# ThibHlln/smartpy

Measured on AMD Instinct MI355X. Metric: MC sample-timesteps/sec/GPU; 1e5 LHS x hourly 10-yr forcing, higher is better.
Workload: dtype f64

## Files before the change

include/smart_amd.h:

```cpp
#ifndef SMART_AMD_H
#define SMART_AMD_H

#include <stdint.h>

#ifdef __cplusplus
extern "C" {
#endif

#define SMART_AMD_ABI_VERSION 7

#define SMART_REPORT_SUMMARY 1
#define SMART_REPORT_RAW 2

#define SMART_MATH_LITERAL 0
#define SMART_MATH_FAST 1

#define SMART_OK 0
#define SMART_E_NULL (-1)
#define SMART_E_SIZE (-2)
#define SMART_E_REPORT_TYPE (-3)
#define SMART_E_WARMUP (-4)
#define SMART_E_GAP (-5)
#define SMART_E_NO_DEVICE (-6)
#define SMART_E_MODE (-7)
// ... 7 lines not shown
#define SMART_PLAN_FORCING_VARYING 0x20
#define SMART_PLAN_FORCING_RUNS 0x80
#define SMART_PLAN_ROWS_ORDERED 0x40
#define SMART_PLAN_VALID 0x100
#define SMART_PLAN_ILLCOND_BLOCKS_SHIFT 12
#define SMART_PLAN_ILLCOND_BLOCKS_MAX 0x7ffff

#define SMART_LITERAL_FORM_AUTO 0
#define SMART_LITERAL_FORM_ROWS 1
#define SMART_LITERAL_FORM_LANES 2

#define SMART_STATUS_SLICE_TIMEOUT 0x1
#define SMART_STATUS_STALE_PLAN 0x2
#define SMART_STATUS_NONFINITE_FORCING 0x4

typedef struct SmartEnsemble {
    int64_t n_catchments;
    int64_t n_samples;
    int64_t n_steps;
    int64_t n_warm;
    int64_t report_gap;
    int32_t report_type;
    int32_t math_mode;
    double delta_sec;

    const double *area_m2;
    const double *forcing;
    const double *params;
    int64_t params_catchment_stride;
    const double *extra;
// ... 2 lines not shown
    const double *gw_obs;

    double *discharge;
    int64_t discharge_ld;
    double *gw;
    double *objfn;
    double *final_vars;
    void *workspace;
    int64_t workspace_bytes;

    void *stream;

    int32_t time_slices;
    int32_t plan;
    int32_t literal_form;
    int32_t reserved0;
} SmartEnsemble;

int64_t smart_n_reports(int64_t n_steps, int64_t report_gap, int32_t report_type);

int smart_run_ensemble_hip(const SmartEnsemble *e);

int smart_check_ensemble(const SmartEnsemble *e);

int64_t smart_workspace_bytes(const SmartEnsemble *e);

int smart_plan_ensemble(const SmartEnsemble *e, int32_t *plan);

int smart_launch_status(const SmartEnsemble *e, int32_t *status);

int smart_describe_launch(const SmartEnsemble *e, char *text, int64_t len);

int smart_allsteps_hip(double area_m2, double delta_sec, int64_t length_simu, const double *nd_rain,
                       const double *nd_peva, const double *nd_parameters, const double *nd_initial,
                       int32_t report_type, int64_t report_gap, double *discharge,
                       double *groundwater_component, double *final_vars);

int smart_hook_counters(int64_t *counters, int64_t n);
// ... 160 lines not shown
```

smartpy_amd/_lib.py:

```python
import contextlib
import ctypes
import os

_HERE = os.path.dirname(os.path.abspath(__file__))
LIB_PATH = os.environ.get('SMART_AMD_LIB') or os.path.join(_HERE, 'csrc', 'libsmart_amd.so')

REPORT_SUMMARY, REPORT_RAW = 1, 2
MATH_LITERAL, MATH_FAST = 0, 1
ABI_VERSION = 7
PLAN_VALID = 0x100
PLAN_CLASS_BITS = {0: 0x01, 1: 0x02, 2: 0x04, 3: 0x08}
PLAN_FORCING_PIECEWISE, PLAN_FORCING_VARYING, PLAN_FORCING_RUNS = 0x10, 0x20, 0x80
PLAN_ROWS_ORDERED = 0x40
PLAN_ILLCOND_BLOCKS_SHIFT, PLAN_ILLCOND_BLOCKS_MAX = 12, 0x7ffff
LITERAL_FORM_AUTO, LITERAL_FORM_ROWS, LITERAL_FORM_LANES = 0, 1, 2
STATUS_SLICE_TIMEOUT, STATUS_STALE_PLAN, STATUS_NONFINITE_FORCING = 0x1, 0x2, 0x4
QUANTILES_AUTO, QUANTILES_SORT, QUANTILES_SELECT = 0, 1, 2
QUANTILES_MAX_PROBS = 16
TRANSFORMS = {'none': 0, 'sqrt': 1, 'log': 2, 'inverse': 3}
OBJFN_WINDOW_COLS = 7
FDC_METHODS = {'auto': 0, 'sort': 1, 'select': 2}
SIGNATURE_NAMES = ['MEAN', 'BFI', 'FLASHINESS', 'AC1', 'RLD', 'RECESSION', 'PEAK', 'PEAK_ROW', 'HIGH_COUNT',
                   'HIGH_DURATION', 'LOW_COUNT', 'LOW_DURATION']
SIGNATURE_COLS = len(SIGNATURE_NAMES)
BOOT_MEAN, BOOT_STD = 0, 1
SOBOL_MAX_PARAMS = 16
PARETO_MAX_OBJECTIVES = 16
PARETO_DIRECTIONS = {'max': 0, 'min': 1, 'target': 2}
ENSEMBLE_SCORE_NAMES = ['CRPS', 'SPREAD', 'PIT_LOW', 'PIT_HIGH', 'MEAN']
ENSEMBLE_SCORE_COLS = len(ENSEMBLE_SCORE_NAMES)
ENSEMBLE_METHODS = {'auto': 0, 'lds': 1, 'global': 2}
# ... 3 lines not shown
PAWN_METHODS = {'auto': 0, 'lds': 1, 'global': 2}

_dp = ctypes.c_void_p


class SmartEnsemble(ctypes.Structure):
    _fields_ = [
        ('n_catchments', ctypes.c_int64), ('n_samples', ctypes.c_int64), ('n_steps', ctypes.c_int64),
        ('n_warm', ctypes.c_int64), ('report_gap', ctypes.c_int64),
        ('report_type', ctypes.c_int32), ('math_mode', ctypes.c_int32), ('delta_sec', ctypes.c_double),
        ('area_m2', _dp), ('forcing', _dp), ('params', _dp), ('params_catchment_stride', ctypes.c_int64),
        ('extra', _dp), ('initial', _dp), ('obs', _dp), ('gw_obs', _dp),
        ('discharge', _dp), ('discharge_ld', ctypes.c_int64), ('gw', _dp), ('objfn', _dp),
        ('final_vars', _dp), ('workspace', _dp), ('workspace_bytes', ctypes.c_int64), ('stream', _dp),
        ('time_slices', ctypes.c_int32), ('plan', ctypes.c_int32),
        ('literal_form', ctypes.c_int32), ('reserved0', ctypes.c_int32),
    ]


SYMBOLS = {
    'smart_n_reports': (ctypes.c_int64, [ctypes.c_int64, ctypes.c_int64, ctypes.c_int32]),
    'smart_run_ensemble_hip': (ctypes.c_int, [ctypes.POINTER(SmartEnsemble)]),
    'smart_check_ensemble': (ctypes.c_int, [ctypes.POINTER(SmartEnsemble)]),
    'smart_workspace_bytes': (ctypes.c_int64, [ctypes.POINTER(SmartEnsemble)]),
    'smart_plan_ensemble': (ctypes.c_int, [ctypes.POINTER(SmartEnsemble), ctypes.POINTER(ctypes.c_int32)]),
    'smart_launch_status': (ctypes.c_int, [ctypes.POINTER(SmartEnsemble), ctypes.POINTER(ctypes.c_int32)]),
    'smart_describe_launch': (ctypes.c_int, [ctypes.POINTER(SmartEnsemble), ctypes.c_char_p, ctypes.c_int64]),
    'smart_allsteps_hip': (ctypes.c_int, [ctypes.c_double, ctypes.c_double, ctypes.c_int64, _dp, _dp, _dp, _dp,
                                          ctypes.c_int32, ctypes.c_int64, _dp, _dp, _dp]),
    'smart_hook_counters': (ctypes.c_int, [ctypes.POINTER(ctypes.c_int64), ctypes.c_int64]),
    'smart_onestep_hip': (ctypes.c_int, [ctypes.c_int64, _dp, _dp]),
    'smart_river_step_hip': (ctypes.c_int, [ctypes.c_int64, _dp, _dp]),
    'smart_objfn_hip': (ctypes.c_int, [ctypes.c_int64, ctypes.c_int64, _dp, ctypes.c_int64, _dp, _dp,
                                       ctypes.c_double, _dp, _dp]),
    'smart_weighted_quantiles_hip': (ctypes.c_int, [ctypes.c_int64, ctypes.c_int64, _dp, ctypes.c_int64, _dp,
                                                    ctypes.POINTER(ctypes.c_double), ctypes.c_int32, _dp,
                                                    ctypes.c_int32, _dp]),
    'smart_quantiles_sort_capacity': (ctypes.c_int64, []),
# ... 122 lines not shown
```

smartpy_amd/csrc/smart_capi.hip:

```cpp
#include "smart_capi_internal.h"
#include "smart_fast_entry.h"

#include <cmath>
#include <cstdarg>
#include <cstdio>
#include <cstdlib>
#include <cstring>
#include <mutex>
#include <vector>

namespace smart {

static_assert(kStatusSliceTimeout == SMART_STATUS_SLICE_TIMEOUT && kStatusStalePlan == SMART_STATUS_STALE_PLAN,
              "status bits of smart_device.h and include/smart_amd.h");

static thread_local char g_err[512] = "";

int fail(int code, const char *fmt, ...)
{
    va_list ap;
    va_start(ap, fmt);
    vsnprintf(g_err, sizeof(g_err), fmt, ap);
    va_end(ap);
    return code;
// ... 55 lines not shown
                    r[4 * j] = f[t].x;
                    r[4 * j + 1] = f[t].y;
                    r[4 * j + 2] = obs && dev && rr >= 0 && rr < a.R ? obs[rr] : 0.0;
                    r[4 * j + 3] = obs && dev && rr >= 0 && rr < a.R ? dev[rr] : 0.0;
                }
                code = a.gap == 1 ? every_code(p, step_kind(f[2 * p]), step_kind(f[2 * p + 1]))
                                  : gap_code(p, a.gap, step_kind(f[2 * p]), step_kind(f[2 * p + 1]));
            }
            for (int j = 0; j < 8; ++j)
                rec[p * 8 + j] = r[j];
            codes[p] = code;
        }
    }
    if (bad)
        __hip_atomic_fetch_or(a.fflags + blockIdx.y, bad, __ATOMIC_RELAXED, __HIP_MEMORY_SCOPE_AGENT);
    if (wild && a.hdr)
        __hip_atomic_fetch_or(a.hdr + kHdrStatus, kStatusNonFiniteForcing, __ATOMIC_RELAXED, __HIP_MEMORY_SCOPE_AGENT);
}

__global__ void smart_workspace_reset(int *hdr, long n_hdr, int *flags, long n_flags)
{
    const long i = (long)blockIdx.x * blockDim.x + threadIdx.x;
    if (i < n_hdr)
        hdr[i] = 0;
    if (i < n_flags)
        flags[i] = 0;
}

__global__ __launch_bounds__(kWave) void smart_classify_rows(KArgs a)
{
    const int cls = wave_class(a, (long)blockIdx.x, (long)blockIdx.y);
    if (threadIdx.x == 0) {
        __hip_atomic_fetch_or(a.hdr + kHdrPlan, 1 << cls, __ATOMIC_RELAXED, __HIP_MEMORY_SCOPE_AGENT);
        if (cls == 3)
            __hip_atomic_fetch_add(a.hdr + kHdrPlanIllCond, 1, __ATOMIC_RELAXED, __HIP_MEMORY_SCOPE_AGENT);
    }
}

__global__ void smart_classify_forcing(KArgs a, int *hdr)
{
    const long c = (long)blockIdx.x * blockDim.x + threadIdx.x;
    if (c < a.n_catch) {
        const int kind = forcing_kind(a, a.fflags[c]);
        __hip_atomic_fetch_or(hdr + kHdrPlan,
                              kind == kForcingIntervals ? SMART_PLAN_FORCING_PIECEWISE
                                                        : (kind == kForcingRuns ? SMART_PLAN_FORCING_RUNS
                                                                                : SMART_PLAN_FORCING_VARYING),
                              __ATOMIC_RELAXED, __HIP_MEMORY_SCOPE_AGENT);
    }
}

constexpr int kMaxDevices = 64, kMaxTodo = 8, kMaxAux = kMaxTodo - 1;

struct DeviceCtx {
    std::once_flag once;
    int n_simd = 0;
    std::mutex mu;
    hipStream_t aux[kMaxAux] = {};
    hipEvent_t fork = nullptr, join[kMaxAux] = {};
    size_t lds_size[kNumFastKernels][17] = {};
    bool lds_known[kNumFastKernels][17] = {};
};

static DeviceCtx g_dev[kMaxDevices];

static DeviceCtx *device_ctx()
{
    int dev = 0;
    if (hipGetDevice(&dev) != hipSuccess || dev < 0 || dev >= kMaxDevices)
        return nullptr;
    DeviceCtx *d = &g_dev[dev];
    std::call_once(d->once, [d, dev] {
        int cus = 0;
        if (hipDeviceGetAttribute(&cus, hipDeviceAttributeMultiprocessorCount, dev) == hipSuccess && cus > 0)
            d->n_simd = cus * 4;
    });
// ... 181 lines not shown
    if (e->params_catchment_stride != 0 && e->params_catchment_stride < e->n_samples * 10)
        return fail(SMART_E_SIZE, "params_catchment_stride must be 0 or >= n_samples * 10");
    if (e->discharge && e->discharge_ld < e->n_samples)
        return fail(SMART_E_SIZE, "discharge_ld must be >= n_samples");
    if (e->objfn && (!e->obs || !e->workspace))
        return fail(SMART_E_NULL, "objfn needs obs and workspace");
    if (e->objfn && e->workspace_bytes < (int64_t)layout(e, false).state_off)
        return fail(SMART_E_SIZE, "workspace_bytes %lld is less than the %lld the header and the observation statistics need",
                    (long long)e->workspace_bytes, (long long)layout(e, false).state_off);
    if (e->time_slices < 0)
        return fail(SMART_E_SIZE, "time_slices must be >= 0");
    if (e->plan != 0 && !(e->plan & SMART_PLAN_VALID))
        return fail(SMART_E_SIZE, "plan must be 0 or a value returned by smart_plan_ensemble");
    if (e->literal_form < SMART_LITERAL_FORM_AUTO || e->literal_form > SMART_LITERAL_FORM_LANES)
        return fail(SMART_E_MODE, "literal_form must be SMART_LITERAL_FORM_AUTO, _ROWS or _LANES");
    clear_error();
    return SMART_OK;
}

int device_ready()
{
    int n = 0;
    hipError_t err = hipGetDeviceCount(&n);
    if (err != hipSuccess)
        return hip_fail(err, "hipGetDeviceCount");
    if (n < 1)
        return fail(SMART_E_NO_DEVICE, "no HIP device is visible; this engine has no CPU fallback");
    return SMART_OK;
}

// ... 94 lines not shown
    a.initial = e->initial;
    a.obs = e->obs;
    a.gw_obs = e->gw_obs;
    a.ws = e->objfn ? w.stats : nullptr;
    a.discharge = e->discharge;
    a.ld = e->discharge_ld;
    a.gw = e->gw;
    a.objfn = e->objfn;
    a.final_vars = e->final_vars;
    a.np_mean = e->math_mode == SMART_MATH_LITERAL && e->report_type == SMART_REPORT_SUMMARY && a.gap >= 8 && a.gap <= 128;
    a.pair_stride = e->final_vars ? (int)kPairStrideSplit : (int)kPairStride;
    a.n_catch = e->n_catchments;
    a.n_blocks = (a.N + kWave - 1) / kWave;
    a.seg_blocks = a.n_blocks * a.n_catch;
    a.hdr = w.hdr;
    a.fflags = nullptr;
    const int merged = merged_report(e);
    if ((merged == kReportMean || merged == kReportLast) && a.gap <= 0x7fffffff) {
        for (long q = 1; q * q <= a.gap && a.n_div < kMaxDiv; ++q)
            if (a.gap % q == 0 && a.gap / q >= 2)
                a.div[a.n_div++] = (int)(a.gap / q);
        for (long q = (long)std::sqrt((double)a.gap) + 1; q >= 2 && a.n_div < kMaxDiv; --q)
            if (q * q < a.gap && a.gap % q == 0 && q < a.div[a.n_div - 1])
                a.div[a.n_div++] = (int)q;
    }
    return a;
}

static void reset_workspace(const Workspace &w, long n_catch, int *flags, long n_flags, hipStream_t s)
{
    const long n_hdr = kHdrInts + n_catch, n = n_hdr > n_flags ? n_hdr : n_flags;
    hipLaunchKernelGGL(smart_workspace_reset, dim3((unsigned)((n + 255) / 256)), dim3(256), 0, s, w.hdr, n_hdr, flags,
                       n_flags);
}

static void set_codes(KArgs *a, const Workspace &w, const Overrides &ov)
{
    a->codes = nullptr, a->estream = nullptr, a->ecodes = nullptr;
    if (!w.codes || !pair_blocks_wanted(ov))
        return;
    if (w.lay.ecodes_off != w.lay.codes_off) {
        a->estream = (const double *)w.codes;
        a->ecodes = (const unsigned *)(w.codes + (w.lay.ecodes_off - w.lay.codes_off));
    } else {
        a->codes = (const uint2 *)w.codes;
    }
}

static void scan_forcing(const SmartEnsemble *e, KArgs a, const Workspace &w, const Overrides &ov, hipStream_t s)
{
    a.fflags = w.fflags;
    set_codes(&a, w, ov);
    hipLaunchKernelGGL(smart_forcing_scan, dim3(64, (unsigned)e->n_catchments), dim3(256), 0, s, a,
                       reinterpret_cast<const double2 *>(e->forcing));
}

static hipError_t launch_kernel(FastKernel k, KArgs a, dim3 grid, size_t lds, hipStream_t s)
{
    const double2 *forcing = reinterpret_cast<const double2 *>(a.forcing);
    const double *obs = a.obs, *ws = a.ws;
    void *args[] = {&a, &forcing, &obs, &ws};
    return hipLaunchKernel(kFastKernels[k].handle, grid, dim3(kWave), args, lds, s);
}

struct Decision {
    FastKernel todo[kMaxTodo];
    int n_todo = 0;
    bool overflow = false;
    void push(FastKernel k)
// ... 86 lines not shown
        return fail(SMART_E_SIZE, "the plan names no class of rows");
    return SMART_OK;
}

static int run(const SmartEnsemble *e, const Overrides &ov, bool literal_rows = false)
{
    int rc = check(e);
    if (rc)
        return rc;
    if ((rc = device_ready()))
        return rc;
    hipStream_t s = (hipStream_t)e->stream;
    const Workspace w = carve(e, ov);
    KArgs a = kernel_args(e, w);

    if (e->objfn)
        hipLaunchKernelGGL(smart_obs_prepare, dim3((unsigned)e->n_catchments), dim3(256), 0, s, e->obs, a.R, w.stats);

    const dim3 grid((unsigned)a.n_blocks, (unsigned)e->n_catchments);
    if (e->math_mode == SMART_MATH_LITERAL) {
        if (w.hdr)
            reset_workspace(w, e->n_catchments, nullptr, 0, s);
        a.hdr = nullptr;
        launch_literal(a, grid, a.np_mean ? (size_t)a.gap * kWave * sizeof(double) : 0, s, literal_rows);
        HIP_TRY(hipGetLastError());
        return SMART_OK;
    }

    DeviceCtx *d = device_ctx();
    if (!d)
        return fail(SMART_E_NO_DEVICE, "cannot query the current HIP device");
    Decision x;
    if ((rc = decide(e, d, w, ov, &x)))
        return rc;
    const int n_seg = x.n_seg, n_todo = x.n_todo;
    a.exits = x.exits;
    a.class_mask = x.class_mask;
    a.pc_mask = x.pc_mask;

    KArgs a_sliced = a;
    if (n_seg > 1) {
        a_sliced.n_seg = n_seg;
        a_sliced.taper = ov.taper && slice_taper_applies(a.W / a.gap + a.R, n_seg);
        a_sliced.seg_state = (double *)w.state;
        a_sliced.seg_flag = (int *)(w.state + (w.lay.flags_off - w.lay.state_off));
        a_sliced.max_polls = ov.max_polls;
        a_sliced.debug_drop = ov.drop_slice;
#ifdef SMART_SLICE_TIMELINE
        a_sliced.timeline = (unsigned long long *)w.timeline;
#endif
    }
    if (w.hdr) {
        reset_workspace(w, e->n_catchments, a_sliced.seg_flag, n_seg > 1 ? a.seg_blocks : 0, s);
        scan_forcing(e, a, w, ov, s);
        if (x.report >= 0 && (x.class_mask & SMART_PLAN_CLASS_REGULAR)) {
            a.fflags = a_sliced.fflags = w.fflags;
            set_codes(&a, w, ov);
            a_sliced.codes = a.codes, a_sliced.estream = a.estream, a_sliced.ecodes = a.ecodes;
        }
    }

    std::lock_guard<std::mutex> lock(d->mu);
    auto launch = [&](FastKernel k, hipStream_t st) -> hipError_t {
        if (kFastKernels[k].sliced && n_seg > 1) {
            const size_t lds = x.per_simd <= 3 ? lds_for_residency(d, k, 4 * x.per_simd) : 0;
            return launch_kernel(k, a_sliced, dim3((unsigned)(a.seg_blocks * n_seg), 1), lds, st);
        }
        return launch_kernel(k, a, dim3(grid.x * kFastKernels[k].waves, grid.y), 0, st);
    };
// ... 70 lines not shown
static int make_plan(const SmartEnsemble *e, const Overrides &ov, int32_t *plan)
{
    if (!plan)
        return fail(SMART_E_NULL, "smart_plan_ensemble: plan is NULL");
    *plan = 0;
    int rc = check(e);
    if (rc)
        return rc;
    if ((rc = device_ready()))
        return rc;
    const Workspace w = carve(e, ov);
    if (!w.hdr)
        return fail(SMART_E_NULL, "smart_plan_ensemble needs a workspace of smart_workspace_bytes() bytes");
    hipStream_t s = (hipStream_t)e->stream;
    KArgs a = kernel_args(e, w);
    reset_workspace(w, e->n_catchments, nullptr, 0, s);
    hipLaunchKernelGGL(smart_classify_rows, dim3((unsigned)a.n_blocks, (unsigned)e->n_catchments), dim3(kWave), 0, s, a);
    if (merged_report(e) == kReportMean || merged_report(e) == kReportLast) {
        scan_forcing(e, a, w, ov, s);
        a.fflags = w.fflags;
        hipLaunchKernelGGL(smart_classify_forcing, dim3((unsigned)((e->n_catchments + 255) / 256)), dim3(256), 0, s,
                           a, w.hdr);
    }
    HIP_TRY(hipGetLastError());
    int bits[2] = {0, 0};
    static_assert(kHdrPlanIllCond == kHdrPlan + 1, "read back together");
    HIP_TRY(hipMemcpyAsync(bits, w.hdr + kHdrPlan, sizeof(bits), hipMemcpyDeviceToHost, s));
    HIP_TRY(hipStreamSynchronize(s));
    const long n_ill = bits[1] < 0 ? 0 : (bits[1] > SMART_PLAN_ILLCOND_BLOCKS_MAX ? SMART_PLAN_ILLCOND_BLOCKS_MAX : bits[1]);
    *plan = SMART_PLAN_VALID | (bits[0] & (0x3f | SMART_PLAN_FORCING_RUNS)) |
            (int32_t)(n_ill << SMART_PLAN_ILLCOND_BLOCKS_SHIFT);
    return SMART_OK;
}

static int launch_status(const SmartEnsemble *e, int32_t *status)
{
    if (!e || !status)
        return fail(SMART_E_NULL, "smart_launch_status: NULL argument");
    *status = 0;
    if (!e->workspace || e->workspace_bytes < (int64_t)layout(e, false).header)
        return SMART_OK;
    int rc = device_ready();
    if (rc)
        return rc;
    int word = 0;
    HIP_TRY(hipMemcpyAsync(&word, (const int *)e->workspace + kHdrStatus, sizeof(int), hipMemcpyDeviceToHost,
// ... 217 lines not shown
}

using namespace smart;

extern "C" {

int64_t smart_n_reports(int64_t n_steps, int64_t report_gap, int32_t report_type)
{
    if (report_gap < 1 || n_steps < 0)
        return 0;
    return report_type == SMART_REPORT_RAW ? (n_steps + report_gap - 1) / report_gap : n_steps / report_gap;
}

int smart_check_ensemble(const SmartEnsemble *e) { return check(e); }

int64_t smart_workspace_bytes(const SmartEnsemble *e) { return workspace_bytes(e, read_overrides()); }

int smart_run_ensemble_hip(const SmartEnsemble *e) { return run(e, read_overrides()); }

int smart_plan_ensemble(const SmartEnsemble *e, int32_t *plan) { return make_plan(e, read_overrides(), plan); }

int smart_launch_status(const SmartEnsemble *e, int32_t *status) { return launch_status(e, status); }

int smart_describe_launch(const SmartEnsemble *e, char *text, int64_t len)
{
    return describe(e, read_overrides(), text, len);
}

int smart_allsteps_hip(double area_m2, double delta_sec, int64_t length_simu, const double *nd_rain,
                       const double *nd_peva, const double *nd_parameters, const double *nd_initial,
// ... 106 lines not shown
```

smartpy_amd/csrc/smart_device.h:

```cpp
#pragma once

#include "smart_slice_cuts.h"
#include "smart_matrix_common.h"

#include <hip/hip_runtime.h>

#include <type_traits>

namespace smart {

constexpr int kMaxDiv = 12;
constexpr int kForcingInsane = 1 << 30;

struct KArgs {
    long N, T, W, gap, R, first_len;
    int report_type;
    int np_mean;
    double dt;
    const double *area;
    const double *forcing;
    const double *params;
    long pstride_c;
    const double *extra;
    const double *initial;
// ... 13 lines not shown
    const double *estream = nullptr;
    const unsigned *ecodes = nullptr;
    int pair_stride = 0;
    const uint2 *codes = nullptr;
    int n_div = 0;
    int div[kMaxDiv] = {};
    int n_seg = 1;
    int taper = 0;
    long n_catch = 1;
    long n_blocks = 0;
    long seg_blocks = 0;
    double *seg_state = nullptr;
    int *seg_flag = nullptr;
    long max_polls = 0;
    int debug_drop = 0;
#ifdef SMART_SLICE_TIMELINE
    unsigned long long *timeline = nullptr;
#endif
};
#ifdef SMART_SLICE_TIMELINE
constexpr int kTimelineFields = 5, kTimelineSlices = 64;
__device__ __forceinline__ void timeline_note(const KArgs &a, long block, long c, int seg, int field,
                                              unsigned long long value)
{
    if (a.timeline && a.n_seg > 1 && seg < kTimelineSlices && seg < a.n_seg && threadIdx.x == 0)
        a.timeline[((long)seg * a.seg_blocks + c * a.n_blocks + block) * kTimelineFields + field] = value;
}
#endif

enum SegField : int {
// ... 2 lines not shown
    kSegPend = 15,
    kSegOutflows = 16,
    kSegA = 17,
    kSegB,
    kSegC1,
    kSegC2,
    kSegC3,
    kSegShift,
    kSegFields
};
enum HdrInt : int {
    kHdrStatus = 0,
    kHdrTicket = 1,
    kHdrPlan = 8,
    kHdrPlanIllCond = 9,
    kHdrInts = 64
};
constexpr int kStatusSliceTimeout = 1, kStatusStalePlan = 2, kStatusNonFiniteForcing = 4;

__device__ __forceinline__ void raise_status(const KArgs &a, int bit)
{
    if (a.hdr && threadIdx.x == 0)
        __hip_atomic_fetch_or(a.hdr + kHdrStatus, bit, __ATOMIC_RELAXED, __HIP_MEMORY_SCOPE_AGENT);
}

#define SMART_NOPS_0 ""
#define SMART_NOPS_1 "s_nop 0\n\t"
#define SMART_NOPS_2 SMART_NOPS_1 SMART_NOPS_1
#define SMART_NOPS_4 SMART_NOPS_2 SMART_NOPS_2
#define SMART_NOPS_8 SMART_NOPS_4 SMART_NOPS_4
// ... 524 lines not shown
                add_moments(val, e, w);
        }
    }
};

template <class Model>
__device__ __forceinline__ void write_results(const KArgs &a, const LaneCtx &x, const Model &m, const Reporter &rep,
                                              double gw, const double *flows = nullptr)
{
    if (x.live)
        a.gw[x.c * a.N + x.n] = gw;
    if (rep.want_obj && x.live) {
        double o[8];
        finish_objectives(rep.ws, rep.A, rep.B, rep.C1, rep.C2, rep.C3, gw, a.gw_obs ? a.gw_obs[x.c] : quiet_nan(),
                          o);
        double *op = a.objfn + (x.c * a.N + x.n) * 8;
#pragma unroll
        for (int i = 0; i < 8; ++i)
            op[i] = o[i];
    }
    if (a.final_vars) {
        double v[19];
        m.get_vars(v, flows);
        if (x.live) {
            double *fp = a.final_vars + (x.c * a.N + x.n) * 19;
#pragma unroll
            for (int i = 0; i < 19; ++i)
                fp[i] = v[i];
        }
    }
}

template <class Model, bool NP_MEAN>
__device__ __forceinline__ void run_ensemble(const KArgs &a, const double2 *__restrict__ forcing,
// ... 444 lines not shown
    [[maybe_unused]] const double *__restrict__ dev_c = ws_all ? ws_all + x.c * (kWsHead + a.R) + kWsHead : nullptr;
    [[maybe_unused]] const uint2 *codes_c = a.codes ? a.codes + x.c * code_chunks(a.T) : nullptr;
    [[maybe_unused]] const double2 *f_asm = reinterpret_cast<const double2 *>(a.forcing) + x.c * a.T;
    double num = 0.0, den = 0.0, q_out_total = 0.0;
    [[maybe_unused]] double num_raw = 0.0, den_raw = 0.0;
    double *hand = a.seg_state + (slot * kSegFields) * kWave + x.lane;
    if (seg > 0) {
        if (!wait_for_slice(a, slot, seg)) {
            const double nan = quiet_nan();
            if (a.discharge && x.live)
                for (long r = ra; r < rb; ++r)
                    a.discharge[(x.c * a.R + r) * a.ld + x.n] = nan;
            if (last) {
                if (x.live) {
                    a.gw[x.c * a.N + x.n] = nan;
                    if (a.objfn)
                        for (int i = 0; i < 8; ++i)
                            a.objfn[(x.c * a.N + x.n) * 8 + i] = nan;
                    if (a.final_vars)
                        for (int i = 0; i < 19; ++i)
                            a.final_vars[(x.c * a.N + x.n) * 19 + i] = nan;
                }
            } else {
                publish_slice(a, slot, seg, false);
            }
            return;
        }
#ifdef SMART_SLICE_TIMELINE
        timeline_note(a, block, catchment, seg, 3, __builtin_amdgcn_s_memrealtime());
#endif
        m.load_state(hand, kWave);
        if constexpr (REPORT == kReportLast) {
            num_raw = hand[kSegOutflows * kWave];
// ... 354 lines not shown
```

smartpy_amd/distributed.py:

```python
import os
import threading
import time
from datetime import timedelta

import torch
import torch.distributed as dist



def shard_bounds(n_rows, world_size, rank):
    per = -(-n_rows // world_size)
    lo = min(rank * per, n_rows)
    return lo, min(lo + per, n_rows)


def shard_counts(n_rows, world_size):
    return [shard_bounds(n_rows, world_size, r)[1] - shard_bounds(n_rows, world_size, r)[0]
            for r in range(world_size)]


def env_world():
    return (int(os.environ.get('RANK', '0')), int(os.environ.get('WORLD_SIZE', '1')),
            int(os.environ.get('LOCAL_RANK', '0')))

# ... 237 lines not shown

class ShardedEnsemble(object):

    def __init__(self, params, forcing, area_m2, delta_sec, n_warm, report_gap, axis='samples', n_catchments=None,
                 obs=None, gw_obs=None, extra=None, device=None, local_block=False, **kw):
        import numpy as np
        from . import engine
        rank, world = rank_world()
        self.axis = axis
        self.device = torch.device(device) if device is not None else engine.default_device()
        if axis == 'samples':
            self.n_total = params.shape[0] * (world if local_block else 1)
            lo, hi = (0, params.shape[0]) if local_block else shard_bounds(self.n_total, world, rank)
            self.n_local = hi - lo
            local_params = params[lo:hi] if hi > lo else params[:1]
            self._prep = engine.prepare_ensemble(local_params, forcing, area_m2, delta_sec, n_warm, report_gap,
                                                 obs=obs, gw_obs=gw_obs, extra=extra, device=self.device, **kw)
            n_run = local_params.shape[0]
            tail = (9,)
        elif axis == 'catchments':
            C = int(n_catchments if n_catchments is not None else forcing.shape[0])
            self.n_total = C
            lo, hi = shard_bounds(C, world, rank)
            self.n_local = hi - lo
            cs = list(range(lo, hi)) if hi > lo else [0]

            def per_catchment(x, shared_ndim):
                if x is None or isinstance(x, dict) or np.ndim(x) <= shared_ndim:
                    return x
                return x[cs]
            f_local = np.stack([np.asarray(forcing(c), dtype=np.float64) for c in cs]) if callable(forcing) \
                else forcing[cs]
            self._prep = engine.prepare_ensemble(
                per_catchment(params, 2), f_local, per_catchment(area_m2, 0), delta_sec, n_warm, report_gap,
                obs=per_catchment(obs, 1), gw_obs=per_catchment(gw_obs, 0), extra=per_catchment(extra, 1),
                device=self.device, **kw)
            n_run = len(cs)
            tail = (params.shape[-2], 9)
        else:
            raise Exception("axis must be 'samples' or 'catchments'")
        per = -(-self.n_total // world)
        self._packed = torch.full((max(per, n_run),) + tail, float('nan'), dtype=torch.float64, device=self.device)
        self._n_run = n_run
        self._gathered = torch.empty((world * per,) + tail, dtype=torch.float64, device=self.device) \
            if is_distributed() and not _host_staged() else None

    def step(self):
        self._prep.enqueue()
        return self._pack_and_gather(self._prep.result())

    def _pack_and_gather(self, out):
        k = self.n_local
        if k:
            if self.axis == 'samples':
                if out.objfn is not None:
                    self._packed[:k, :8].copy_(out.objfn[:k])
                self._packed[:k, 8].copy_(out.gw[:k])
            else:
                objfn = out.objfn if out.objfn is None or out.objfn.dim() == 3 else out.objfn.unsqueeze(0)
                gw = out.gw if out.gw.dim() == 2 else out.gw.unsqueeze(0)
                if objfn is not None:
                    self._packed[:k, :, :8].copy_(objfn[:k])
                self._packed[:k, :, 8].copy_(gw[:k])
        per = -(-self.n_total // rank_world()[1])
        return gather_rows(self._packed[:per], self.n_total, out=self._gathered)

    def verify(self):
        from .engine import SmartEngineError
# ... 42 lines not shown
```

smartpy_amd/engine.py:

```python
import collections
import ctypes
import math
import threading
import warnings
import weakref

import numpy as np
import torch

from . import _lib
from ._lib import SmartEngineError, REPORT_SUMMARY, REPORT_RAW, MATH_LITERAL, MATH_FAST

OBJ_FN_NAMES = ['NSE', 'KGE', 'KGEc', 'KGEa', 'KGEb', 'PBias', 'RMSE', 'GW']
VARIABLES = ['Q_aeva', 'Q_ove', 'Q_dra', 'Q_int', 'Q_sgw', 'Q_dgw', 'Q_out',
             'V_ove', 'V_dra', 'V_int', 'V_sgw', 'V_dgw',
             'V_ly1', 'V_ly2', 'V_ly3', 'V_ly4', 'V_ly5', 'V_ly6', 'V_river']

_REPORT = {'summary': REPORT_SUMMARY, 'raw': REPORT_RAW}
_MATH = {'literal': MATH_LITERAL, 'fast': MATH_FAST}
_LITERAL_FORMS = {'auto': _lib.LITERAL_FORM_AUTO, 'rows': _lib.LITERAL_FORM_ROWS, 'lanes': _lib.LITERAL_FORM_LANES}


def report_code(report):
    try:
# ... 161 lines not shown
def _compose_plan(planned, keep=0, row_class=None):
    if row_class is not None:
        forcing = _lib.PLAN_FORCING_PIECEWISE | _lib.PLAN_FORCING_VARYING | _lib.PLAN_FORCING_RUNS
        return _lib.PLAN_VALID | (planned & forcing) | _lib.PLAN_CLASS_BITS[row_class]
    return planned | (keep & _lib.PLAN_ROWS_ORDERED)


class PreparedEnsemble(object):

    repeated = False

    def __init__(self, e, device, n_samples, squeeze, outputs, workspace, grouping, caller_out, keep, memo):
        self._e = e
        self.device, self.n_samples, self._squeeze = device, n_samples, squeeze
        self._dis, self._gw, self._objfn, self._fin = outputs
        self._ws = workspace
        self._grouping = grouping
        self._caller_out = caller_out
        self._keep = keep
        self._memo = memo

    @property
    def has_status(self):
        return self._ws is not None and self._e.math_mode == MATH_FAST

    def enqueue(self):
        with torch.cuda.device(self.device):
            self._e.stream = torch.cuda.current_stream(self.device).cuda_stream
            _lib.check(_lib.lib().smart_run_ensemble_hip(ctypes.byref(self._e)))

    def launch(self):
        self.enqueue()
        return self._result()

    def result(self):
        return self._result()

    def status(self):
        word = ctypes.c_int32(0)
        with torch.cuda.device(self.device):
            self._e.stream = torch.cuda.current_stream(self.device).cuda_stream
            _lib.check(_lib.lib().smart_launch_status(ctypes.byref(self._e), ctypes.byref(word)))
        return int(word.value)

# ... 12 lines not shown
            word, ' + '.join(n for b, n in ((_lib.STATUS_SLICE_TIMEOUT, 'a time slice timed out'),
                                            (_lib.STATUS_STALE_PLAN, 'stale plan'),
                                            (_lib.STATUS_NONFINITE_FORCING, 'a NaN or an infinity in the forcing'))
                             if word & b),
            'in literal arithmetic' if word & _lib.STATUS_NONFINITE_FORCING else (
                'without time slices' if word & _lib.STATUS_SLICE_TIMEOUT else 'with a fresh plan')))
        if word & _lib.STATUS_NONFINITE_FORCING:
            self._e.math_mode = MATH_LITERAL
        if word & _lib.STATUS_SLICE_TIMEOUT:
            self._e.time_slices = 1
        if word & _lib.STATUS_STALE_PLAN:
            self._memo.forget()
            self._memo.refresh()
            self._plan()
            self._memo.store((self._grouping, int(self._e.plan)))
        self.enqueue()
        word = self.status()
        if word != 0:
            raise SmartEngineError(-6, "smartpy_amd: the repeated launch reports status %#x as well" % word)
        return self._result()

    def _plan(self, ordered=0):
        keep, word = self._e.plan | ordered, ctypes.c_int32(0)
        self._e.plan = 0
        with torch.cuda.device(self.device):
            self._e.stream = torch.cuda.current_stream(self.device).cuda_stream
            _lib.check(_lib.lib().smart_plan_ensemble(ctypes.byref(self._e), ctypes.byref(word)))
        self._e.plan = _compose_plan(int(word.value), keep)

    def aim_at(self, row_class):
        self._e.plan = _compose_plan(self._e.plan, row_class=row_class)

    def _result(self):
        dis, gw, objfn, fin = self._dis, self._gw, self._objfn, self._fin
        if self._grouping is not None:
            inverse = self._grouping[1]
            gw = gw[:, inverse]
            objfn = None if objfn is None else objfn[:, inverse]
            fin = None if fin is None else fin[:, inverse]
# ... 21 lines not shown
        raise Exception("params [C, N, 10] must have one block per catchment")
    if params.shape[-1] != 10:
        raise Exception("params must have 10 columns (T, C, H, D, S, Z, SK, FK, GK, RK)")
    pstride = 0 if params.dim() == 2 else params.shape[1] * 10
    rtype = report_code(report)
    try:
        mmode = _MATH[math_mode]
    except KeyError:
        raise Exception("math mode '{}' unknown.".format(math_mode))
    if mmode == MATH_FAST and not (isinstance(forcing_in, torch.Tensor) and forcing_in.is_cuda):
        if not bool(np.isfinite(np.asarray(forcing_in, dtype=np.float64)).all()):
            mmode = MATH_LITERAL
    return device, params, forcing, squeeze, pstride, rtype, mmode


def _allocate_outputs(C, R, N, device, want_discharge, want_objfn, want_final, discharge_out):
    dis = discharge_out
    if dis is not None:
        assert dis.is_contiguous() and dis.dtype == torch.float64 and dis.shape[:2] == (C, R) and dis.shape[2] >= N
    elif want_discharge:
        dis = torch.empty((C, R, N), dtype=torch.float64, device=device)
    return (dis, torch.empty((C, N), dtype=torch.float64, device=device),
            torch.empty((C, N, 8), dtype=torch.float64, device=device) if want_objfn else None,
            torch.empty((C, N, 19), dtype=torch.float64, device=device) if want_final else None)


def _fill_struct(inputs, outputs, pstride, n_warm, report_gap, rtype, mmode, delta_sec, time_slices, literal_form):
    def ptr(t):
        return None if t is None else t.data_ptr()

    forcing, params, dis = inputs[1], inputs[2], outputs[0]
    e = _lib.SmartEnsemble()
    e.n_catchments, e.n_samples, e.n_steps, e.n_warm = forcing.shape[0], params.shape[-2], forcing.shape[1], int(n_warm)
    e.report_gap, e.report_type, e.math_mode, e.delta_sec = int(report_gap), rtype, mmode, float(delta_sec)
    e.area_m2, e.forcing, e.params, e.extra, e.initial, e.obs, e.gw_obs = [ptr(t) for t in inputs]
    e.discharge, e.gw, e.objfn, e.final_vars = [ptr(t) for t in outputs]
    e.discharge_ld = params.shape[-2] if dis is None else dis.shape[2]
    e.params_catchment_stride, e.time_slices = pstride, int(time_slices)
    try:
        e.literal_form = _LITERAL_FORMS[literal_form]
    except KeyError:
        raise Exception("literal_form '{}' unknown ('auto', 'rows' or 'lanes').".format(literal_form))
    return e


def _size_workspace(e, device):
    with torch.cuda.device(device):
        n_ws = int(_lib.lib().smart_workspace_bytes(ctypes.byref(e)))
    ws = torch.empty((n_ws + 7) // 8, dtype=torch.float64, device=device) if n_ws > 0 else None
    e.workspace, e.workspace_bytes = (None if ws is None else ws.data_ptr()), n_ws
    _lib.check(_lib.lib().smart_check_ensemble(ctypes.byref(e)))
    return ws


def prepare_ensemble(params, forcing, area_m2, delta_sec, n_warm, report_gap, report='summary', extra=None,
                     initial=None, obs=None, gw_obs=None, math_mode='fast', want_discharge=True, want_objfn=None,
                     want_final=False, device=None, discharge_out=None, group_variants=True, time_slices=0,
                     literal_form='auto'):
    _lib.lib()
    inputs_in = (params, forcing)
    device, params, forcing, squeeze, pstride, rtype, mmode = _normalise_inputs(params, forcing, report, math_mode, device)
    C, T, N = forcing.shape[0], forcing.shape[1], params.shape[-2]
    R = n_reports(T, report_gap, rtype)
    area = _per_catchment(area_m2, device, C)
    extra = _per_catchment(extra_vector(extra) if isinstance(extra, dict) else extra, device, C, (7,))
    initial = _per_catchment(initial, device, C, (N, 12))
    if want_objfn is None:
        want_objfn = obs is not None
    if want_objfn and obs is None:
        raise Exception("objective functions need observations")
    obs = _per_catchment(obs, device, C, (R,))
    gw_obs = _per_catchment(gw_obs, device, C)

    sort_rows = not want_discharge and discharge_out is None
    memo = _Memo(inputs_in, (float(delta_sec), int(report_gap), rtype, C, N, T, bool(group_variants), sort_rows),
                 device, initial, mmode == MATH_FAST)
    known = memo.lookup()
    grouping, caller_out = None, None
    if group_variants and mmode == MATH_FAST and pstride == 0 and N > 64:
        grouping = known[0] if known else _variant_grouping(params, float(delta_sec), sort_rows, initial, area)
    if grouping is not None:
        params = params[grouping[0]].contiguous()
        initial = None if initial is None else initial[:, grouping[0]].contiguous()
    if grouping is not None and discharge_out is not None:
        caller_out, discharge_out, want_discharge = discharge_out, None, True
    outputs = _allocate_outputs(C, R, params.shape[-2], device, want_discharge, want_objfn, want_final, discharge_out)
    inputs = (area, forcing, params, extra, initial, obs, gw_obs)
    e = _fill_struct(inputs, outputs, pstride, n_warm, report_gap, rtype, mmode, delta_sec, time_slices, literal_form)
    p = PreparedEnsemble(e, device, N, squeeze, outputs, _size_workspace(e, device), grouping, caller_out, inputs, memo)
    if p.has_status:
        if known:
            e.plan = known[1]
        elif not torch.cuda.is_current_stream_capturing():
            p._plan(_lib.PLAN_ROWS_ORDERED if (sort_rows and grouping is not None) else 0)
            memo.store((grouping, int(e.plan)))
    return p


def run_ensemble(params, forcing, area_m2, delta_sec, n_warm, report_gap, report='summary', extra=None,
                 initial=None, obs=None, gw_obs=None, math_mode='fast', want_discharge=True, want_objfn=None,
                 want_final=False, device=None, discharge_out=None, group_variants=True, time_slices=0, verify=True,
                 literal_form='auto'):
    p = prepare_ensemble(params, forcing, area_m2, delta_sec, n_warm, report_gap, report=report, extra=extra,
                         initial=initial, obs=obs, gw_obs=gw_obs, math_mode=math_mode,
                         want_discharge=want_discharge, want_objfn=want_objfn, want_final=want_final, device=device,
                         discharge_out=discharge_out, group_variants=group_variants, time_slices=time_slices,
                         literal_form=literal_form)
    p.enqueue()
    out = p.verify() if verify and p.has_status and not torch.cuda.is_current_stream_capturing() else p.result()
    out._prepared = p
# ... 93 lines not shown
```

Measured before the change: 957.0 billion.

## Cache forcing scan and obs preparation across launches; write packed results directly

Adds a prepare-inputs entry point that runs the observation preparation and forcing scan once and records them per workspace. Later launches skip those kernels when forcing and obs have not changed, and the nonfinite-forcing status is carried in a kept header slot. Separately, a packed-results flag lets the kernel write objectives plus groundwater into a 9-wide caller buffer, so the distributed gather no longer needs its copy step. The cost is extra host bookkeeping and the risk of stale cached state if inputs change without a version bump.

```diff
diff --git a/include/smart_amd.h b/include/smart_amd.h
--- a/include/smart_amd.h
+++ b/include/smart_amd.h
@@ -45,6 +45,9 @@
 #define SMART_STATUS_STALE_PLAN 0x2
 #define SMART_STATUS_NONFINITE_FORCING 0x4
 
+#define SMART_LAUNCH_INPUTS_PREPARED 0x1
+#define SMART_LAUNCH_PACKED_RESULTS 0x2
+
 typedef struct SmartEnsemble {
     int64_t n_catchments;
     int64_t n_samples;
@@ -77,7 +80,7 @@
     int32_t time_slices;
     int32_t plan;
     int32_t literal_form;
-    int32_t reserved0;
+    int32_t launch_flags;
 } SmartEnsemble;
 
 int64_t smart_n_reports(int64_t n_steps, int64_t report_gap, int32_t report_type);
@@ -85,6 +88,8 @@
 int smart_run_ensemble_hip(const SmartEnsemble *e);
 
 int smart_check_ensemble(const SmartEnsemble *e);
+
+int smart_prepare_inputs(const SmartEnsemble *e);
 
 int64_t smart_workspace_bytes(const SmartEnsemble *e);
 
diff --git a/smartpy_amd/_lib.py b/smartpy_amd/_lib.py
--- a/smartpy_amd/_lib.py
+++ b/smartpy_amd/_lib.py
@@ -15,6 +15,7 @@
 PLAN_ILLCOND_BLOCKS_SHIFT, PLAN_ILLCOND_BLOCKS_MAX = 12, 0x7ffff
 LITERAL_FORM_AUTO, LITERAL_FORM_ROWS, LITERAL_FORM_LANES = 0, 1, 2
 STATUS_SLICE_TIMEOUT, STATUS_STALE_PLAN, STATUS_NONFINITE_FORCING = 0x1, 0x2, 0x4
+LAUNCH_INPUTS_PREPARED, LAUNCH_PACKED_RESULTS = 0x1, 0x2
 QUANTILES_AUTO, QUANTILES_SORT, QUANTILES_SELECT = 0, 1, 2
 QUANTILES_MAX_PROBS = 16
 TRANSFORMS = {'none': 0, 'sqrt': 1, 'log': 2, 'inverse': 3}
@@ -48,7 +49,7 @@
         ('discharge', _dp), ('discharge_ld', ctypes.c_int64), ('gw', _dp), ('objfn', _dp),
         ('final_vars', _dp), ('workspace', _dp), ('workspace_bytes', ctypes.c_int64), ('stream', _dp),
         ('time_slices', ctypes.c_int32), ('plan', ctypes.c_int32),
-        ('literal_form', ctypes.c_int32), ('reserved0', ctypes.c_int32),
+        ('literal_form', ctypes.c_int32), ('launch_flags', ctypes.c_int32),
     ]
 
 
@@ -56,6 +57,7 @@
     'smart_n_reports': (ctypes.c_int64, [ctypes.c_int64, ctypes.c_int64, ctypes.c_int32]),
     'smart_run_ensemble_hip': (ctypes.c_int, [ctypes.POINTER(SmartEnsemble)]),
     'smart_check_ensemble': (ctypes.c_int, [ctypes.POINTER(SmartEnsemble)]),
+    'smart_prepare_inputs': (ctypes.c_int, [ctypes.POINTER(SmartEnsemble)]),
     'smart_workspace_bytes': (ctypes.c_int64, [ctypes.POINTER(SmartEnsemble)]),
     'smart_plan_ensemble': (ctypes.c_int, [ctypes.POINTER(SmartEnsemble), ctypes.POINTER(ctypes.c_int32)]),
     'smart_launch_status': (ctypes.c_int, [ctypes.POINTER(SmartEnsemble), ctypes.POINTER(ctypes.c_int32)]),
diff --git a/smartpy_amd/csrc/smart_capi.hip b/smartpy_amd/csrc/smart_capi.hip
--- a/smartpy_amd/csrc/smart_capi.hip
+++ b/smartpy_amd/csrc/smart_capi.hip
@@ -93,15 +93,17 @@
     }
     if (bad)
         __hip_atomic_fetch_or(a.fflags + blockIdx.y, bad, __ATOMIC_RELAXED, __HIP_MEMORY_SCOPE_AGENT);
-    if (wild && a.hdr)
+    if (wild && a.hdr) {
         __hip_atomic_fetch_or(a.hdr + kHdrStatus, kStatusNonFiniteForcing, __ATOMIC_RELAXED, __HIP_MEMORY_SCOPE_AGENT);
-}
-
-__global__ void smart_workspace_reset(int *hdr, long n_hdr, int *flags, long n_flags)
+        __hip_atomic_fetch_or(a.hdr + kHdrKept, kStatusNonFiniteForcing, __ATOMIC_RELAXED, __HIP_MEMORY_SCOPE_AGENT);
+    }
+}
+
+__global__ void smart_workspace_reset(int *hdr, long n_hdr, int *flags, long n_flags, int prepared)
 {
     const long i = (long)blockIdx.x * blockDim.x + threadIdx.x;
-    if (i < n_hdr)
-        hdr[i] = 0;
+    if (i < n_hdr && !(prepared && i == kHdrKept))
+        hdr[i] = prepared && i == kHdrStatus ? hdr[kHdrKept] : 0;
     if (i < n_flags)
         flags[i] = 0;
 }
@@ -131,6 +133,23 @@
 
 constexpr int kMaxDevices = 64, kMaxTodo = 8, kMaxAux = kMaxTodo - 1;
 
+struct PreparedInputs {
+    const void *workspace = nullptr;
+    const void *forcing = nullptr, *obs = nullptr;
+    const void *stats = nullptr, *codes = nullptr, *ecodes = nullptr;
+    long C = 0, T = 0, R = 0, gap = 0;
+    int report_type = 0, pair_stride = 0;
+    int merged = 0;
+    int form = 0;
+    bool same(const PreparedInputs &o) const
+    {
+        return workspace == o.workspace && forcing == o.forcing && obs == o.obs && stats == o.stats && codes == o.codes &&
+               ecodes == o.ecodes && C == o.C && T == o.T && R == o.R && gap == o.gap && report_type == o.report_type &&
+               pair_stride == o.pair_stride && merged == o.merged && form == o.form;
+    }
+};
+constexpr int kMaxPrepared = 16;
+
 struct DeviceCtx {
     std::once_flag once;
     int n_simd = 0;
@@ -139,6 +158,32 @@
     hipEvent_t fork = nullptr, join[kMaxAux] = {};
     size_t lds_size[kNumFastKernels][17] = {};
     bool lds_known[kNumFastKernels][17] = {};
+    PreparedInputs prepared[kMaxPrepared];
+    int next_prepared = 0;
+    bool is_prepared(const PreparedInputs &p) const
+    {
+        for (const PreparedInputs &q : prepared)
+            if (q.workspace && q.same(p))
+                return true;
+        return false;
+    }
+    void forget_prepared(const void *workspace)
+    {
+        for (PreparedInputs &q : prepared)
+            if (q.workspace == workspace)
+                q = PreparedInputs();
+    }
+    void note_prepared(const PreparedInputs &p)
+    {
+        forget_prepared(p.workspace);
+        for (PreparedInputs &q : prepared)
+            if (!q.workspace) {
+                q = p;
+                return;
+            }
+        prepared[next_prepared] = p;
+        next_prepared = (next_prepared + 1) % kMaxPrepared;
+    }
 };
 
 static DeviceCtx g_dev[kMaxDevices];
@@ -350,6 +395,11 @@
         return fail(SMART_E_SIZE, "plan must be 0 or a value returned by smart_plan_ensemble");
     if (e->literal_form < SMART_LITERAL_FORM_AUTO || e->literal_form > SMART_LITERAL_FORM_LANES)
         return fail(SMART_E_MODE, "literal_form must be SMART_LITERAL_FORM_AUTO, _ROWS or _LANES");
+    if (e->launch_flags & ~(SMART_LAUNCH_INPUTS_PREPARED | SMART_LAUNCH_PACKED_RESULTS))
+        return fail(SMART_E_MODE, "launch_flags %#x holds bits this library does not know (SMART_LAUNCH_*)",
+                    (unsigned)e->launch_flags);
+    if ((e->launch_flags & SMART_LAUNCH_PACKED_RESULTS) && !e->objfn)
+        return fail(SMART_E_NULL, "SMART_LAUNCH_PACKED_RESULTS needs objfn");
     clear_error();
     return SMART_OK;
 }
@@ -474,6 +524,7 @@
     a.n_blocks = (a.N + kWave - 1) / kWave;
     a.seg_blocks = a.n_blocks * a.n_catch;
     a.hdr = w.hdr;
+    a.packed = (e->launch_flags & SMART_LAUNCH_PACKED_RESULTS) != 0;
     a.fflags = nullptr;
     const int merged = merged_report(e);
     if ((merged == kReportMean || merged == kReportLast) && a.gap <= 0x7fffffff) {
@@ -487,11 +538,12 @@
     return a;
 }
 
-static void reset_workspace(const Workspace &w, long n_catch, int *flags, long n_flags, hipStream_t s)
-{
-    const long n_hdr = kHdrInts + n_catch, n = n_hdr > n_flags ? n_hdr : n_flags;
+static void reset_workspace(const Workspace &w, long n_catch, int *flags, long n_flags, hipStream_t s,
+                            bool prepared = false)
+{
+    const long n_hdr = prepared ? kHdrInts : kHdrInts + n_catch, n = n_hdr > n_flags ? n_hdr : n_flags;
     hipLaunchKernelGGL(smart_workspace_reset, dim3((unsigned)((n + 255) / 256)), dim3(256), 0, s, w.hdr, n_hdr, flags,
-                       n_flags);
+                       n_flags, prepared ? 1 : 0);
 }
 
 static void set_codes(KArgs *a, const Workspace &w, const Overrides &ov)
@@ -513,6 +565,31 @@
     set_codes(&a, w, ov);
     hipLaunchKernelGGL(smart_forcing_scan, dim3(64, (unsigned)e->n_catchments), dim3(256), 0, s, a,
                        reinterpret_cast<const double2 *>(e->forcing));
+}
+
+static PreparedInputs prepared_inputs_of(const SmartEnsemble *e, KArgs a, const Workspace &w, const Overrides &ov)
+{
+    set_codes(&a, w, ov);
+    PreparedInputs p;
+    p.workspace = e->workspace;
+    p.forcing = e->forcing;
+    p.obs = e->obs;
+    p.stats = a.ws;
+    p.codes = a.codes ? (const void *)a.codes : (const void *)a.estream;
+    p.ecodes = a.ecodes;
+    p.C = a.n_catch, p.T = a.T, p.R = a.R, p.gap = a.gap;
+    p.report_type = a.report_type, p.pair_stride = a.pair_stride;
+    p.merged = merged_report(e);
+    p.form = a.codes ? 1 : (a.estream ? 2 : 0);
+    return p;
+}
+
+static void prepare_inputs(const SmartEnsemble *e, const KArgs &a, const Workspace &w, const Overrides &ov, hipStream_t s)
+{
+    if (e->objfn)
+        hipLaunchKernelGGL(smart_obs_prepare, dim3((unsigned)e->n_catchments), dim3(256), 0, s, e->obs, a.R, w.stats);
+    reset_workspace(w, e->n_catchments, nullptr, 0, s);
+    scan_forcing(e, a, w, ov, s);
 }
 
 static hipError_t launch_kernel(FastKernel k, KArgs a, dim3 grid, size_t lds, hipStream_t s)
@@ -629,7 +706,17 @@
     const Workspace w = carve(e, ov);
     KArgs a = kernel_args(e, w);
 
-    if (e->objfn)
+    DeviceCtx *d = device_ctx();
+    bool prepared = false;
+    if (d && w.hdr) {
+        std::lock_guard<std::mutex> lock(d->mu);
+        prepared = e->math_mode == SMART_MATH_FAST && (e->launch_flags & SMART_LAUNCH_INPUTS_PREPARED) &&
+                   d->is_prepared(prepared_inputs_of(e, a, w, ov));
+        if (!prepared)
+            d->forget_prepared(e->workspace);
+    }
+
+    if (e->objfn && !prepared)
         hipLaunchKernelGGL(smart_obs_prepare, dim3((unsigned)e->n_catchments), dim3(256), 0, s, e->obs, a.R, w.stats);
 
     const dim3 grid((unsigned)a.n_blocks, (unsigned)e->n_catchments);
@@ -642,7 +729,6 @@
         return SMART_OK;
     }
 
-    DeviceCtx *d = device_ctx();
     if (!d)
         return fail(SMART_E_NO_DEVICE, "cannot query the current HIP device");
     Decision x;
@@ -666,8 +752,9 @@
 #endif
     }
     if (w.hdr) {
-        reset_workspace(w, e->n_catchments, a_sliced.seg_flag, n_seg > 1 ? a.seg_blocks : 0, s);
-        scan_forcing(e, a, w, ov, s);
+        reset_workspace(w, e->n_catchments, a_sliced.seg_flag, n_seg > 1 ? a.seg_blocks : 0, s, prepared);
+        if (!prepared)
+            scan_forcing(e, a, w, ov, s);
         if (x.report >= 0 && (x.class_mask & SMART_PLAN_CLASS_REGULAR)) {
             a.fflags = a_sliced.fflags = w.fflags;
             set_codes(&a, w, ov);
@@ -768,6 +855,10 @@
         return fail(SMART_E_NULL, "smart_plan_ensemble needs a workspace of smart_workspace_bytes() bytes");
     hipStream_t s = (hipStream_t)e->stream;
     KArgs a = kernel_args(e, w);
+    if (DeviceCtx *d = device_ctx()) {
+        std::lock_guard<std::mutex> lock(d->mu);
+        d->forget_prepared(e->workspace);
+    }
     reset_workspace(w, e->n_catchments, nullptr, 0, s);
     hipLaunchKernelGGL(smart_classify_rows, dim3((unsigned)a.n_blocks, (unsigned)e->n_catchments), dim3(kWave), 0, s, a);
     if (merged_report(e) == kReportMean || merged_report(e) == kReportLast) {
@@ -784,6 +875,32 @@
     const long n_ill = bits[1] < 0 ? 0 : (bits[1] > SMART_PLAN_ILLCOND_BLOCKS_MAX ? SMART_PLAN_ILLCOND_BLOCKS_MAX : bits[1]);
     *plan = SMART_PLAN_VALID | (bits[0] & (0x3f | SMART_PLAN_FORCING_RUNS)) |
             (int32_t)(n_ill << SMART_PLAN_ILLCOND_BLOCKS_SHIFT);
+    return SMART_OK;
+}
+
+static int prepare(const SmartEnsemble *e, const Overrides &ov)
+{
+    int rc = check(e);
+    if (rc)
+        return rc;
+    if (e->math_mode != SMART_MATH_FAST)
+        return SMART_OK;
+    if ((rc = device_ready()))
+        return rc;
+    const Workspace w = carve(e, ov);
+    DeviceCtx *d = device_ctx();
+    if (!w.hdr || !d)
+        return !d ? fail(SMART_E_NO_DEVICE, "cannot query the current HIP device")
+                  : fail(SMART_E_NULL, "smart_prepare_inputs needs a workspace of smart_workspace_bytes() bytes");
+    const KArgs a = kernel_args(e, w);
+    {
+        std::lock_guard<std::mutex> lock(d->mu);
+        d->forget_prepared(e->workspace);
+    }
+    prepare_inputs(e, a, w, ov, (hipStream_t)e->stream);
+    HIP_TRY(hipGetLastError());
+    std::lock_guard<std::mutex> lock(d->mu);
+    d->note_prepared(prepared_inputs_of(e, a, w, ov));
     return SMART_OK;
 }
 
@@ -1031,6 +1148,8 @@
 
 int smart_check_ensemble(const SmartEnsemble *e) { return check(e); }
 
+int smart_prepare_inputs(const SmartEnsemble *e) { return prepare(e, read_overrides()); }
+
 int64_t smart_workspace_bytes(const SmartEnsemble *e) { return workspace_bytes(e, read_overrides()); }
 
 int smart_run_ensemble_hip(const SmartEnsemble *e) { return run(e, read_overrides()); }
diff --git a/smartpy_amd/csrc/smart_device.h b/smartpy_amd/csrc/smart_device.h
--- a/smartpy_amd/csrc/smart_device.h
+++ b/smartpy_amd/csrc/smart_device.h
@@ -51,6 +51,7 @@
     int *seg_flag = nullptr;
     long max_polls = 0;
     int debug_drop = 0;
+    int packed = 0;
 #ifdef SMART_SLICE_TIMELINE
     unsigned long long *timeline = nullptr;
 #endif
@@ -83,6 +84,7 @@
     kHdrTicket = 1,
     kHdrPlan = 8,
     kHdrPlanIllCond = 9,
+    kHdrKept = 10,
     kHdrInts = 64
 };
 constexpr int kStatusSliceTimeout = 1, kStatusStalePlan = 2, kStatusNonFiniteForcing = 4;
@@ -637,10 +639,12 @@
         double o[8];
         finish_objectives(rep.ws, rep.A, rep.B, rep.C1, rep.C2, rep.C3, gw, a.gw_obs ? a.gw_obs[x.c] : quiet_nan(),
                           o);
-        double *op = a.objfn + (x.c * a.N + x.n) * 8;
+        double *op = a.objfn + (x.c * a.N + x.n) * (a.packed ? 9 : 8);
 #pragma unroll
         for (int i = 0; i < 8; ++i)
             op[i] = o[i];
+        if (a.packed)
+            op[8] = gw;
     }
     if (a.final_vars) {
         double v[19];
@@ -1115,9 +1119,11 @@
             if (last) {
                 if (x.live) {
                     a.gw[x.c * a.N + x.n] = nan;
-                    if (a.objfn)
-                        for (int i = 0; i < 8; ++i)
-                            a.objfn[(x.c * a.N + x.n) * 8 + i] = nan;
+                    if (a.objfn) {
+                        const int wide = a.packed ? 9 : 8;
+                        for (int i = 0; i < wide; ++i)
+                            a.objfn[(x.c * a.N + x.n) * wide + i] = nan;
+                    }
                     if (a.final_vars)
                         for (int i = 0; i < 19; ++i)
                             a.final_vars[(x.c * a.N + x.n) * 19 + i] = nan;
diff --git a/smartpy_amd/distributed.py b/smartpy_amd/distributed.py
--- a/smartpy_amd/distributed.py
+++ b/smartpy_amd/distributed.py
@@ -275,10 +275,11 @@
             lo, hi = (0, params.shape[0]) if local_block else shard_bounds(self.n_total, world, rank)
             self.n_local = hi - lo
             local_params = params[lo:hi] if hi > lo else params[:1]
+            n_run = local_params.shape[0]
+            self._allocate(n_run, (9,), world)
             self._prep = engine.prepare_ensemble(local_params, forcing, area_m2, delta_sec, n_warm, report_gap,
-                                                 obs=obs, gw_obs=gw_obs, extra=extra, device=self.device, **kw)
-            n_run = local_params.shape[0]
-            tail = (9,)
+                                                 obs=obs, gw_obs=gw_obs, extra=extra, device=self.device,
+                                                 packed_out=self._packed if hi > lo else None, **kw)
         elif axis == 'catchments':
             C = int(n_catchments if n_catchments is not None else forcing.shape[0])
             self.n_total = C
@@ -292,14 +293,16 @@
                 return x[cs]
             f_local = np.stack([np.asarray(forcing(c), dtype=np.float64) for c in cs]) if callable(forcing) \
                 else forcing[cs]
+            n_run = len(cs)
+            self._allocate(n_run, (params.shape[-2], 9), world)
             self._prep = engine.prepare_ensemble(
                 per_catchment(params, 2), f_local, per_catchment(area_m2, 0), delta_sec, n_warm, report_gap,
                 obs=per_catchment(obs, 1), gw_obs=per_catchment(gw_obs, 0), extra=per_catchment(extra, 1),
-                device=self.device, **kw)
-            n_run = len(cs)
-            tail = (params.shape[-2], 9)
+                device=self.device, packed_out=self._packed if hi > lo else None, **kw)
         else:
             raise Exception("axis must be 'samples' or 'catchments'")
+
+    def _allocate(self, n_run, tail, world):
         per = -(-self.n_total // world)
         self._packed = torch.full((max(per, n_run),) + tail, float('nan'), dtype=torch.float64, device=self.device)
         self._n_run = n_run
@@ -312,7 +315,7 @@
 
     def _pack_and_gather(self, out):
         k = self.n_local
-        if k:
+        if k and not getattr(self._prep, 'packed', False):
             if self.axis == 'samples':
                 if out.objfn is not None:
                     self._packed[:k, :8].copy_(out.objfn[:k])
diff --git a/smartpy_amd/engine.py b/smartpy_amd/engine.py
--- a/smartpy_amd/engine.py
+++ b/smartpy_amd/engine.py
@@ -199,6 +199,10 @@
         self._e = e
         self.device, self.n_samples, self._squeeze = device, n_samples, squeeze
         self._dis, self._gw, self._objfn, self._fin = outputs
+        self.packed = bool(e.launch_flags & _lib.LAUNCH_PACKED_RESULTS)
+        if self.packed:
+            self._objfn = self._objfn[:, :, :8]
+        self._inputs_at = None
         self._ws = workspace
         self._grouping = grouping
         self._caller_out = caller_out
@@ -212,7 +216,28 @@
     def enqueue(self):
         with torch.cuda.device(self.device):
             self._e.stream = torch.cuda.current_stream(self.device).cuda_stream
+            self._prepare_inputs()
             _lib.check(_lib.lib().smart_run_ensemble_hip(ctypes.byref(self._e)))
+
+    def _prepare_inputs(self):
+        if not self.has_status:
+            return
+        forcing, obs = self._keep[1], self._keep[5]
+        now = (forcing._version, None if obs is None else obs._version)
+        stream = self._e.stream
+        if self._inputs_at != now:
+            self._e.launch_flags &= ~_lib.LAUNCH_INPUTS_PREPARED
+            if torch.cuda.is_current_stream_capturing():
+                return
+            _lib.check(_lib.lib().smart_prepare_inputs(ctypes.byref(self._e)))
+            self._inputs_at = now
+            self._inputs_event = torch.cuda.Event()
+            self._inputs_event.record(torch.cuda.current_stream(self.device))
+            self._inputs_streams = {stream}
+        elif stream not in self._inputs_streams and not torch.cuda.is_current_stream_capturing():
+            torch.cuda.current_stream(self.device).wait_event(self._inputs_event)
+            self._inputs_streams.add(stream)
+        self._e.launch_flags |= _lib.LAUNCH_INPUTS_PREPARED
 
     def launch(self):
         self.enqueue()
@@ -255,6 +280,7 @@
             self._memo.refresh()
             self._plan()
             self._memo.store((self._grouping, int(self._e.plan)))
+        self._inputs_at = None
         self.enqueue()
         word = self.status()
         if word != 0:
@@ -264,6 +290,7 @@
     def _plan(self, ordered=0):
         keep, word = self._e.plan | ordered, ctypes.c_int32(0)
         self._e.plan = 0
+        self._inputs_at = None
         with torch.cuda.device(self.device):
             self._e.stream = torch.cuda.current_stream(self.device).cuda_stream
             _lib.check(_lib.lib().smart_plan_ensemble(ctypes.byref(self._e), ctypes.byref(word)))
@@ -315,14 +342,18 @@
     return device, params, forcing, squeeze, pstride, rtype, mmode
 
 
-def _allocate_outputs(C, R, N, device, want_discharge, want_objfn, want_final, discharge_out):
+def _allocate_outputs(C, R, N, device, want_discharge, want_objfn, want_final, discharge_out, packed_out=None):
     dis = discharge_out
     if dis is not None:
         assert dis.is_contiguous() and dis.dtype == torch.float64 and dis.shape[:2] == (C, R) and dis.shape[2] >= N
     elif want_discharge:
         dis = torch.empty((C, R, N), dtype=torch.float64, device=device)
-    return (dis, torch.empty((C, N), dtype=torch.float64, device=device),
-            torch.empty((C, N, 8), dtype=torch.float64, device=device) if want_objfn else None,
+    objfn = torch.empty((C, N, 8), dtype=torch.float64, device=device) if want_objfn else None
+    if packed_out is not None:
+        assert packed_out.is_contiguous() and packed_out.dtype == torch.float64 and packed_out.shape[-1] == 9
+        assert packed_out.device.type == torch.device(device).type and packed_out.numel() >= C * N * 9
+        objfn = packed_out.view(-1)[:C * N * 9].view(C, N, 9)
+    return (dis, torch.empty((C, N), dtype=torch.float64, device=device), objfn,
             torch.empty((C, N, 19), dtype=torch.float64, device=device) if want_final else None)
 
 
@@ -338,6 +369,8 @@
     e.discharge, e.gw, e.objfn, e.final_vars = [ptr(t) for t in outputs]
     e.discharge_ld = params.shape[-2] if dis is None else dis.shape[2]
     e.params_catchment_stride, e.time_slices = pstride, int(time_slices)
+    if outputs[2] is not None and outputs[2].shape[-1] == 9:
+        e.launch_flags |= _lib.LAUNCH_PACKED_RESULTS
     try:
         e.literal_form = _LITERAL_FORMS[literal_form]
     except KeyError:
@@ -357,7 +390,7 @@
 def prepare_ensemble(params, forcing, area_m2, delta_sec, n_warm, report_gap, report='summary', extra=None,
                      initial=None, obs=None, gw_obs=None, math_mode='fast', want_discharge=True, want_objfn=None,
                      want_final=False, device=None, discharge_out=None, group_variants=True, time_slices=0,
-                     literal_form='auto'):
+                     literal_form='auto', packed_out=None):
     _lib.lib()
     inputs_in = (params, forcing)
     device, params, forcing, squeeze, pstride, rtype, mmode = _normalise_inputs(params, forcing, report, math_mode, device)
@@ -385,7 +418,8 @@
         initial = None if initial is None else initial[:, grouping[0]].contiguous()
     if grouping is not None and discharge_out is not None:
         caller_out, discharge_out, want_discharge = discharge_out, None, True
-    outputs = _allocate_outputs(C, R, params.shape[-2], device, want_discharge, want_objfn, want_final, discharge_out)
+    outputs = _allocate_outputs(C, R, params.shape[-2], device, want_discharge, want_objfn, want_final, discharge_out,
+                                packed_out if grouping is None and want_objfn else None)
     inputs = (area, forcing, params, extra, initial, obs, gw_obs)
     e = _fill_struct(inputs, outputs, pstride, n_warm, report_gap, rtype, mmode, delta_sec, time_slices, literal_form)
     p = PreparedEnsemble(e, device, N, squeeze, outputs, _size_workspace(e, device), grouping, caller_out, inputs, memo)
@@ -395,6 +429,9 @@
         elif not torch.cuda.is_current_stream_capturing():
             p._plan(_lib.PLAN_ROWS_ORDERED if (sort_rows and grouping is not None) else 0)
             memo.store((grouping, int(e.plan)))
+        with torch.cuda.device(device):
+            e.stream = torch.cuda.current_stream(device).cuda_stream
+            p._prepare_inputs()
     return p
 
 
```

After: 963.1 billion (median of 6 runs). Within noise of the previous version (+0.6%).
